# facebookresearch/multimodal

Measured on NVIDIA H100. Metric: image-text pairs/sec (CLIP ViT-B/16 contrastive pretrain step, bs=512/GPU), higher is better.
Workload: dtype bf16

## Files before the change

### multimodal_b200/csrc/attention.cu

```cuda
#include "attention_tiles.cuh"
#include "mmb200_internal.h"
#include <stdlib.h>

namespace mmb {

constexpr int SMAX = 384;

__device__ __forceinline__ void load_tile(uint8_t* dst, const __nv_bfloat16* src, long long ld, int S, int S_pad) {
  for (int i = threadIdx.x; i < S_pad * 8; i += blockDim.x) {
    const int r = i >> 3, ch = i & 7;
    uint4 v = make_uint4(0, 0, 0, 0);
    if (r < S) v = __ldg(reinterpret_cast<const uint4*>(src + (long long)r * ld + ch * 8));
    *reinterpret_cast<uint4*>(dst + toff(r, ch * 8)) = v;
  }
}
__device__ __forceinline__ void cp_tile_rows(uint8_t* dst, const __nv_bfloat16* src, long long ld, int S, int r0,
                                             int r1) {
  for (int i = r0 * 8 + threadIdx.x; i < r1 * 8; i += blockDim.x) {
    const int r = i >> 3, ch = i & 7;
    const bool in = r < S;
    cp_async16(smem_u32(dst + toff(r, ch * 8)), src + (in ? (long long)r * ld + ch * 8 : 0), in ? 16u : 0u);
  }
}

__device__ __forceinline__ void load_keymask(uint8_t* dst, const uint8_t* kmask, int S, int S_pad) {
  for (int i = threadIdx.x; i < S_pad; i += blockDim.x) dst[i] = (i < S && (!kmask || kmask[i])) ? 1 : 0;
}

template <bool CAUSAL>
__global__ void __launch_bounds__(256) attn_fwd_kernel(const __nv_bfloat16* __restrict__ qkv,
                                                       __nv_bfloat16* __restrict__ out, float* __restrict__ lse,
                                                       const uint8_t* __restrict__ kmask, int S, int H,
                                                       float scale_log2) {
  extern __shared__ __align__(128) uint8_t asmem[];
  const int S_pad = (S + 15) & ~15;
  const int d = H * HD;
  const long long ld = 3LL * d;
  const int b = blockIdx.x / H, h = blockIdx.x - b * H;
  uint8_t* sQ = asmem;
  uint8_t* sK = sQ + S_pad * 128;
  uint8_t* sV = sK + S_pad * 128;
  uint64_t* bars = reinterpret_cast<uint64_t*>(sV + S_pad * 128);
  uint8_t* sM = reinterpret_cast<uint8_t*>(bars + SMAX / 64);
  const __nv_bfloat16* base = qkv + (long long)b * S * ld + h * HD;
  const int n_kc = (S_pad + 63) >> 6;
  if (threadIdx.x == 0)
    for (int c = 0; c < n_kc; ++c) mbar_init(&bars[c], blockDim.x);
  load_keymask(sM, kmask ? kmask + (long long)b * S : nullptr, S, S_pad);
  __syncthreads();
  cp_tile_rows(sQ, base, ld, S, 0, S_pad);
  for (int c = 0; c < n_kc; ++c) {
    const int k1 = min(S_pad, (c + 1) * 64);
    cp_tile_rows(sK, base + d, ld, S, c * 64, k1);
    cp_tile_rows(sV, base + 2 * d, ld, S, c * 64, k1);
    cp_async_arrive(&bars[c]);
  }
  const uint32_t uQ = smem_u32(sQ), uK = smem_u32(sK), uV = smem_u32(sV);
  const int warp = threadIdx.x >> 5, lane = threadIdx.x & 31, nwarps = blockDim.x >> 5;
  const int g = lane >> 2, t = lane & 3;
  const int n_qt = S_pad >> 4;
  mbar_wait_quiet(&bars[0], 0);

  for (int qt = warp; qt < n_qt; qt += nwarps) {
    const int q0 = qt * 16;
    uint32_t qa[4][4];
#pragma unroll
    for (int ks = 0; ks < 4; ++ks) load_a(qa[ks], uQ, q0, ks * 16, lane);
    float o[8][4];
#pragma unroll
    for (int i = 0; i < 8; ++i) o[i][0] = o[i][1] = o[i][2] = o[i][3] = 0.f;
    float m0 = -INFINITY, m1 = -INFINITY, l0 = 0.f, l1 = 0.f;
    const int r0 = q0 + g, r1 = r0 + 8;
    const int kv_end = CAUSAL ? min(S, q0 + 16) : S;

    for (int kvb = 0; kvb < kv_end; kvb += 64) {
      mbar_wait_quiet(&bars[kvb >> 6], 0);
      const int nt_valid = min(8, (kv_end - kvb + 7) >> 3);
      float s[8][4];
#pragma unroll
      for (int nt = 0; nt < 8; ++nt) {
        s[nt][0] = s[nt][1] = s[nt][2] = s[nt][3] = 0.f;
        if (nt < nt_valid) {
#pragma unroll
          for (int kp = 0; kp < 2; ++kp) {
            uint32_t kb[4];
            load_b_nk(kb, uK, kvb + nt * 8, kp * 32, lane);
            mma16816(s[nt], qa[2 * kp], kb[0], kb[1]);
            mma16816(s[nt], qa[2 * kp + 1], kb[2], kb[3]);
          }
        }
      }
      float mx0 = -INFINITY, mx1 = -INFINITY;
#pragma unroll
      for (int nt = 0; nt < 8; ++nt) {
#pragma unroll
        for (int e = 0; e < 4; ++e) {
          const int col = kvb + nt * 8 + 2 * t + (e & 1);
          const int row = (e < 2) ? r0 : r1;
          float v = s[nt][e] * scale_log2;
          if (col >= kv_end || !sM[col] || (CAUSAL && col > row)) v = -INFINITY;
          s[nt][e] = v;
        }
        mx0 = fmaxf(mx0, fmaxf(s[nt][0], s[nt][1]));
        mx1 = fmaxf(mx1, fmaxf(s[nt][2], s[nt][3]));
      }
      mx0 = quad_max(mx0);
      mx1 = quad_max(mx1);
      const float mn0 = fmaxf(m0, mx0), mn1 = fmaxf(m1, mx1);
      const float b0 = (mn0 == -INFINITY) ? 0.f : mn0, b1 = (mn1 == -INFINITY) ? 0.f : mn1;
      const float c0 = exp2f(m0 - b0), c1 = exp2f(m1 - b1);
      float rs0 = 0.f, rs1 = 0.f;
#pragma unroll
      for (int nt = 0; nt < 8; ++nt) {
        s[nt][0] = exp2f(s[nt][0] - b0);
        s[nt][1] = exp2f(s[nt][1] - b0);
        s[nt][2] = exp2f(s[nt][2] - b1);
        s[nt][3] = exp2f(s[nt][3] - b1);
        rs0 += s[nt][0] + s[nt][1];
        rs1 += s[nt][2] + s[nt][3];
      }
      l0 = l0 * c0 + rs0;
      l1 = l1 * c1 + rs1;
      m0 = mn0;
      m1 = mn1;
#pragma unroll
      for (int i = 0; i < 8; ++i) {
        o[i][0] *= c0; o[i][1] *= c0; o[i][2] *= c1; o[i][3] *= c1;
      }
#pragma unroll
      for (int ks = 0; ks < 4; ++ks) {
        if (2 * ks < nt_valid) {
          uint32_t pa[4];
          pa[0] = pack_bf16x2(s[2 * ks][0], s[2 * ks][1]);
          pa[1] = pack_bf16x2(s[2 * ks][2], s[2 * ks][3]);
          pa[2] = pack_bf16x2(s[2 * ks + 1][0], s[2 * ks + 1][1]);
          pa[3] = pack_bf16x2(s[2 * ks + 1][2], s[2 * ks + 1][3]);
#pragma unroll
          for (int np = 0; np < 4; ++np) {
            uint32_t vb[4];
            load_b_kn(vb, uV, kvb + ks * 16, np * 16, lane);
            mma16816(o[2 * np], pa, vb[0], vb[1]);
            mma16816(o[2 * np + 1], pa, vb[2], vb[3]);
          }
        }
      }
    }
    l0 = quad_sum(l0);
    l1 = quad_sum(l1);
    const float i0 = l0 > 0.f ? 1.f / l0 : 0.f, i1 = l1 > 0.f ? 1.f / l1 : 0.f;
    __nv_bfloat16* orow0 = out + ((long long)b * S + r0) * d + h * HD;
    __nv_bfloat16* orow1 = out + ((long long)b * S + r1) * d + h * HD;
#pragma unroll
    for (int nt = 0; nt < 8; ++nt) {
      if (r0 < S) *reinterpret_cast<uint32_t*>(orow0 + nt * 8 + 2 * t) = pack_bf16x2(o[nt][0] * i0, o[nt][1] * i0);
      if (r1 < S) *reinterpret_cast<uint32_t*>(orow1 + nt * 8 + 2 * t) = pack_bf16x2(o[nt][2] * i1, o[nt][3] * i1);
    }
    if (lse && t == 0) {
      float* lrow = lse + ((long long)b * H + h) * S;
      if (r0 < S) lrow[r0] = (m0 + log2f(l0)) * 0.6931471805599453f;
      if (r1 < S) lrow[r1] = (m1 + log2f(l1)) * 0.6931471805599453f;
    }
  }
  cp_async_wait_all();
}

template <bool CAUSAL>
__global__ void __launch_bounds__(256) attn_bwd_kernel(const __nv_bfloat16* __restrict__ qkv,
                                                       const __nv_bfloat16* __restrict__ out,
                                                       const __nv_bfloat16* __restrict__ dout,
                                                       const float* __restrict__ lse,
                                                       const uint8_t* __restrict__ kmask,
                                                       __nv_bfloat16* __restrict__ dqkv, int S, int H, float scale) {
  extern __shared__ __align__(128) uint8_t asmem[];
  const int S_pad = (S + 15) & ~15;
  const int d = H * HD;
  const long long ld = 3LL * d;
  const int b = blockIdx.x / H, h = blockIdx.x - b * H;
  uint8_t* sQ = asmem;
  uint8_t* sK = sQ + S_pad * 128;
  uint8_t* sV = sK + S_pad * 128;
  uint8_t* sdO = sV + S_pad * 128;
  float* sL = reinterpret_cast<float*>(sdO + S_pad * 128);
  float* sD = sL + S_pad;
  uint8_t* sM = reinterpret_cast<uint8_t*>(sD + S_pad);
  const __nv_bfloat16* base = qkv + (long long)b * S * ld + h * HD;
  const __nv_bfloat16* obase = out + (long long)b * S * d + h * HD;
  const __nv_bfloat16* dobase = dout + (long long)b * S * d + h * HD;
  load_tile(sQ, base, ld, S, S_pad);
  load_tile(sK, base + d, ld, S, S_pad);
  load_tile(sV, base + 2 * d, ld, S, S_pad);
  load_tile(sdO, dobase, d, S, S_pad);
  load_keymask(sM, kmask ? kmask + (long long)b * S : nullptr, S, S_pad);
  const int warp = threadIdx.x >> 5, lane = threadIdx.x & 31, nwarps = blockDim.x >> 5;
  for (int r = warp; r < S_pad; r += nwarps) {
    float acc = 0.f;
    if (r < S) {
      const uint32_t a = *reinterpret_cast<const uint32_t*>(obase + (long long)r * d + lane * 2);
      const uint32_t c = *reinterpret_cast<const uint32_t*>(dobase + (long long)r * d + lane * 2);
      acc = bf16_lo(a) * bf16_lo(c) + bf16_hi(a) * bf16_hi(c);
    }
#pragma unroll
    for (int o = 16; o > 0; o >>= 1) acc += __shfl_xor_sync(0xffffffffu, acc, o);
    if (lane == 0) {
      sD[r] = acc;
      sL[r] = (r < S) ? lse[((long long)b * H + h) * S + r] * 1.4426950408889634f : 0.f;
    }
  }
  __syncthreads();
  const uint32_t uQ = smem_u32(sQ), uK = smem_u32(sK), uV = smem_u32(sV), uO = smem_u32(sdO);
  const int g = lane >> 2, t = lane & 3;
  const int n_t = S_pad >> 4;
  const float scale_log2 = scale * 1.4426950408889634f;
  __nv_bfloat16* dbase = dqkv + (long long)b * S * ld + h * HD;

  for (int j = warp; j < n_t; j += nwarps) {
    const int kv0 = j * 16;
    uint32_t ka[4][4], va[4][4];
#pragma unroll
    for (int ks = 0; ks < 4; ++ks) {
      load_a(ka[ks], uK, kv0, ks * 16, lane);
      load_a(va[ks], uV, kv0, ks * 16, lane);
    }
    float dk[8][4], dv[8][4];
#pragma unroll
    for (int i = 0; i < 8; ++i) {
      dk[i][0] = dk[i][1] = dk[i][2] = dk[i][3] = 0.f;
      dv[i][0] = dv[i][1] = dv[i][2] = dv[i][3] = 0.f;
    }
    const bool kv_ok0 = sM[kv0 + g] != 0, kv_ok1 = sM[kv0 + g + 8] != 0;
    for (int i = CAUSAL ? j : 0; i < n_t; ++i) {
      const int q0 = i * 16;
      float st[2][4], dpt[2][4];
#pragma unroll
      for (int nt = 0; nt < 2; ++nt) {
        st[nt][0] = st[nt][1] = st[nt][2] = st[nt][3] = 0.f;
        dpt[nt][0] = dpt[nt][1] = dpt[nt][2] = dpt[nt][3] = 0.f;
#pragma unroll
        for (int kp = 0; kp < 2; ++kp) {
          uint32_t qb[4], ob[4];
          load_b_nk(qb, uQ, q0 + nt * 8, kp * 32, lane);
          mma16816(st[nt], ka[2 * kp], qb[0], qb[1]);
          mma16816(st[nt], ka[2 * kp + 1], qb[2], qb[3]);
          load_b_nk(ob, uO, q0 + nt * 8, kp * 32, lane);
          mma16816(dpt[nt], va[2 * kp], ob[0], ob[1]);
          mma16816(dpt[nt], va[2 * kp + 1], ob[2], ob[3]);
        }
      }
      float pT[2][4], dsT[2][4];
#pragma unroll
      for (int nt = 0; nt < 2; ++nt)
#pragma unroll
        for (int e = 0; e < 4; ++e) {
          const int kv = kv0 + g + (e >> 1) * 8;
          const int q = q0 + nt * 8 + 2 * t + (e & 1);
          const bool valid = ((e >> 1) ? kv_ok1 : kv_ok0) && (q < S) && (!CAUSAL || kv <= q);
          const float p = valid ? exp2f(st[nt][e] * scale_log2 - sL[q]) : 0.f;
          pT[nt][e] = p;
          dsT[nt][e] = p * (dpt[nt][e] - sD[q]) * scale;
        }
      uint32_t pa[4], dsa[4];
      pa[0] = pack_bf16x2(pT[0][0], pT[0][1]); pa[1] = pack_bf16x2(pT[0][2], pT[0][3]);
      pa[2] = pack_bf16x2(pT[1][0], pT[1][1]); pa[3] = pack_bf16x2(pT[1][2], pT[1][3]);
      dsa[0] = pack_bf16x2(dsT[0][0], dsT[0][1]); dsa[1] = pack_bf16x2(dsT[0][2], dsT[0][3]);
      dsa[2] = pack_bf16x2(dsT[1][0], dsT[1][1]); dsa[3] = pack_bf16x2(dsT[1][2], dsT[1][3]);
#pragma unroll
      for (int np = 0; np < 4; ++np) {
        uint32_t bb[4];
        load_b_kn(bb, uO, q0, np * 16, lane);
        mma16816(dv[2 * np], pa, bb[0], bb[1]);
        mma16816(dv[2 * np + 1], pa, bb[2], bb[3]);
        load_b_kn(bb, uQ, q0, np * 16, lane);
        mma16816(dk[2 * np], dsa, bb[0], bb[1]);
        mma16816(dk[2 * np + 1], dsa, bb[2], bb[3]);
      }
    }
    const int r0 = kv0 + g, r1 = r0 + 8;
#pragma unroll
    for (int nt = 0; nt < 8; ++nt) {
      if (r0 < S) {
        *reinterpret_cast<uint32_t*>(dbase + (long long)r0 * ld + d + nt * 8 + 2 * t) = pack_bf16x2(dk[nt][0], dk[nt][1]);
        *reinterpret_cast<uint32_t*>(dbase + (long long)r0 * ld + 2 * d + nt * 8 + 2 * t) = pack_bf16x2(dv[nt][0], dv[nt][1]);
      }
      if (r1 < S) {
        *reinterpret_cast<uint32_t*>(dbase + (long long)r1 * ld + d + nt * 8 + 2 * t) = pack_bf16x2(dk[nt][2], dk[nt][3]);
        *reinterpret_cast<uint32_t*>(dbase + (long long)r1 * ld + 2 * d + nt * 8 + 2 * t) = pack_bf16x2(dv[nt][2], dv[nt][3]);
      }
    }
  }

  for (int i = warp; i < n_t; i += nwarps) {
    const int q0 = i * 16;
    uint32_t qa[4][4], oa[4][4];
#pragma unroll
    for (int ks = 0; ks < 4; ++ks) {
      load_a(qa[ks], uQ, q0, ks * 16, lane);
      load_a(oa[ks], uO, q0, ks * 16, lane);
    }
    float dq[8][4];
#pragma unroll
    for (int n = 0; n < 8; ++n) dq[n][0] = dq[n][1] = dq[n][2] = dq[n][3] = 0.f;
    const int r0 = q0 + g, r1 = r0 + 8;
    const float L0 = sL[r0], L1 = sL[r1], D0 = sD[r0], D1 = sD[r1];
    const int j_end = CAUSAL ? i + 1 : n_t;
    for (int j = 0; j < j_end; ++j) {
      const int kv0 = j * 16;
      float s[2][4], dp[2][4];
#pragma unroll
      for (int nt = 0; nt < 2; ++nt) {
        s[nt][0] = s[nt][1] = s[nt][2] = s[nt][3] = 0.f;
        dp[nt][0] = dp[nt][1] = dp[nt][2] = dp[nt][3] = 0.f;
#pragma unroll
        for (int kp = 0; kp < 2; ++kp) {
          uint32_t kb[4], vb[4];
          load_b_nk(kb, uK, kv0 + nt * 8, kp * 32, lane);
          mma16816(s[nt], qa[2 * kp], kb[0], kb[1]);
          mma16816(s[nt], qa[2 * kp + 1], kb[2], kb[3]);
          load_b_nk(vb, uV, kv0 + nt * 8, kp * 32, lane);
          mma16816(dp[nt], oa[2 * kp], vb[0], vb[1]);
          mma16816(dp[nt], oa[2 * kp + 1], vb[2], vb[3]);
        }
      }
      float ds[2][4];
#pragma unroll
      for (int nt = 0; nt < 2; ++nt)
#pragma unroll
        for (int e = 0; e < 4; ++e) {
          const int row = (e < 2) ? r0 : r1;
          const int col = kv0 + nt * 8 + 2 * t + (e & 1);
          const bool valid = (row < S) && sM[col] && (!CAUSAL || col <= row);
          const float p = valid ? exp2f(s[nt][e] * scale_log2 - ((e < 2) ? L0 : L1)) : 0.f;
          ds[nt][e] = p * (dp[nt][e] - ((e < 2) ? D0 : D1)) * scale;
        }
      uint32_t dsa[4];
      dsa[0] = pack_bf16x2(ds[0][0], ds[0][1]); dsa[1] = pack_bf16x2(ds[0][2], ds[0][3]);
      dsa[2] = pack_bf16x2(ds[1][0], ds[1][1]); dsa[3] = pack_bf16x2(ds[1][2], ds[1][3]);
#pragma unroll
      for (int np = 0; np < 4; ++np) {
        uint32_t bb[4];
        load_b_kn(bb, uK, kv0, np * 16, lane);
        mma16816(dq[2 * np], dsa, bb[0], bb[1]);
        mma16816(dq[2 * np + 1], dsa, bb[2], bb[3]);
      }
    }
#pragma unroll
    for (int nt = 0; nt < 8; ++nt) {
      if (r0 < S) *reinterpret_cast<uint32_t*>(dbase + (long long)r0 * ld + nt * 8 + 2 * t) = pack_bf16x2(dq[nt][0], dq[nt][1]);
      if (r1 < S) *reinterpret_cast<uint32_t*>(dbase + (long long)r1 * ld + nt * 8 + 2 * t) = pack_bf16x2(dq[nt][2], dq[nt][3]);
    }
  }
}

constexpr int BWD_STAGED_MAX = 224;
constexpr int BWD_STAGED_THREADS = BWD_STAGED_MAX / 16 * 32;
constexpr int BWD_STAGED_BARS = 1 + (BWD_STAGED_MAX + 63) / 64;

__host__ __device__ constexpr int ds_stride(int S_pad) { return 2 * S_pad + 16; }
__host__ __device__ constexpr int bwd_staged_smem(int S_pad) {
  return 4 * S_pad * 128 + S_pad * ds_stride(S_pad) + 2 * S_pad * 4 + 8 * BWD_STAGED_BARS + S_pad;
}
static_assert(bwd_staged_smem(BWD_STAGED_MAX) <= 227 * 1024, "staged backward exceeds the sm_90 shared-memory opt-in");

template <bool CAUSAL>
__global__ void __launch_bounds__(BWD_STAGED_THREADS, 1) attn_bwd_staged_kernel(
    const __nv_bfloat16* __restrict__ qkv, const __nv_bfloat16* __restrict__ out, const __nv_bfloat16* __restrict__ dout,
    const float* __restrict__ lse, const uint8_t* __restrict__ kmask, __nv_bfloat16* __restrict__ dqkv, int S, int H,
    float scale) {
  extern __shared__ __align__(128) uint8_t asmem[];
  const int S_pad = (S + 15) & ~15;
  const int dstride = ds_stride(S_pad);
  const int d = H * HD;
  const long long ld = 3LL * d;
  const int b = blockIdx.x / H, h = blockIdx.x - b * H;
  uint8_t* sQ = asmem;
  uint8_t* sK = sQ + S_pad * 128;
  uint8_t* sV = sK + S_pad * 128;
  uint8_t* sdO = sV + S_pad * 128;
  uint8_t* sdS = sdO + S_pad * 128;
  float* sL = reinterpret_cast<float*>(sdS + S_pad * dstride);
  float* sD = sL + S_pad;
  uint64_t* bars = reinterpret_cast<uint64_t*>(sD + S_pad);
  uint8_t* sM = reinterpret_cast<uint8_t*>(bars + BWD_STAGED_BARS);
  const __nv_bfloat16* base = qkv + (long long)b * S * ld + h * HD;
  const __nv_bfloat16* obase = out + (long long)b * S * d + h * HD;
  const __nv_bfloat16* dobase = dout + (long long)b * S * d + h * HD;
  const int n_qc = (S_pad + 63) >> 6;
  if (threadIdx.x == 0)
    for (int c = 0; c <= n_qc; ++c) mbar_init(&bars[c], blockDim.x);
  load_keymask(sM, kmask ? kmask + (long long)b * S : nullptr, S, S_pad);
  __syncthreads();
  cp_tile_rows(sK, base + d, ld, S, 0, S_pad);
  cp_tile_rows(sV, base + 2 * d, ld, S, 0, S_pad);
  cp_async_arrive(&bars[0]);
  for (int c = 0; c < n_qc; ++c) {
    const int q1 = min(S_pad, (c + 1) * 64);
    cp_tile_rows(sQ, base, ld, S, c * 64, q1);
    cp_tile_rows(sdO, dobase, d, S, c * 64, q1);
    cp_async_arrive(&bars[1 + c]);
  }
  for (int r = threadIdx.x >> 3; r < S_pad; r += blockDim.x >> 3) {
    const int ch = threadIdx.x & 7;
    float v[4] = {0.f, 0.f, 0.f, 0.f};
    if (r < S) {
      const uint4 a = __ldg(reinterpret_cast<const uint4*>(obase + (long long)r * d + ch * 8));
      const uint4 c = __ldg(reinterpret_cast<const uint4*>(dobase + (long long)r * d + ch * 8));
      v[0] = bf16_lo(a.x) * bf16_lo(c.x) + bf16_hi(a.x) * bf16_hi(c.x);
      v[1] = bf16_lo(a.y) * bf16_lo(c.y) + bf16_hi(a.y) * bf16_hi(c.y);
      v[2] = bf16_lo(a.z) * bf16_lo(c.z) + bf16_hi(a.z) * bf16_hi(c.z);
      v[3] = bf16_lo(a.w) * bf16_lo(c.w) + bf16_hi(a.w) * bf16_hi(c.w);
    }
#pragma unroll
    for (int o = 4; o > 0; o >>= 1)
#pragma unroll
      for (int k = 0; k < 4; ++k) v[k] += __shfl_xor_sync(0xffffffffu, v[k], o);
    if (ch == 0) {
      sD[r] = (v[0] + v[2]) + (v[1] + v[3]);
      sL[r] = (r < S) ? lse[((long long)b * H + h) * S + r] * 1.4426950408889634f : 0.f;
    }
  }
  __syncthreads();
  const uint32_t uQ = smem_u32(sQ), uK = smem_u32(sK), uV = smem_u32(sV), uO = smem_u32(sdO), udS = smem_u32(sdS);
  const int warp = threadIdx.x >> 5, lane = threadIdx.x & 31;
  const int g = lane >> 2, t = lane & 3;
  const int n_t = S_pad >> 4;
  const float scale_log2 = scale * 1.4426950408889634f;
  __nv_bfloat16* dbase = dqkv + (long long)b * S * ld + h * HD;

  {
    const int j = warp, kv0 = j * 16;
    mbar_wait_quiet(&bars[0], 0);
    float dk[8][4], dv[8][4];
#pragma unroll
    for (int i = 0; i < 8; ++i) {
      dk[i][0] = dk[i][1] = dk[i][2] = dk[i][3] = 0.f;
      dv[i][0] = dv[i][1] = dv[i][2] = dv[i][3] = 0.f;
    }
    const bool kv_ok0 = sM[kv0 + g] != 0, kv_ok1 = sM[kv0 + g + 8] != 0;
    const int i0 = CAUSAL ? j : 0;
#pragma unroll 1
    for (int i = i0; i < n_t; ++i) {
      while (!mbar_try_wait(&bars[1 + (i >> 2)], 0)) {}
      const int q0 = i * 16;
      float st[2][4], dpt[2][4];
#pragma unroll
      for (int nt = 0; nt < 2; ++nt) {
        st[nt][0] = st[nt][1] = st[nt][2] = st[nt][3] = 0.f;
        dpt[nt][0] = dpt[nt][1] = dpt[nt][2] = dpt[nt][3] = 0.f;
      }
#pragma unroll
      for (int kp = 0; kp < 2; ++kp) {
        uint32_t ka0[4], ka1[4];
        load_a(ka0, uK, kv0, kp * 32, lane);
        load_a(ka1, uK, kv0, kp * 32 + 16, lane);
#pragma unroll
        for (int nt = 0; nt < 2; ++nt) {
          uint32_t qb[4];
          load_b_nk(qb, uQ, q0 + nt * 8, kp * 32, lane);
          mma16816(st[nt], ka0, qb[0], qb[1]);
          mma16816(st[nt], ka1, qb[2], qb[3]);
        }
      }
#pragma unroll
      for (int kp = 0; kp < 2; ++kp) {
        uint32_t va0[4], va1[4];
        load_a(va0, uV, kv0, kp * 32, lane);
        load_a(va1, uV, kv0, kp * 32 + 16, lane);
#pragma unroll
        for (int nt = 0; nt < 2; ++nt) {
          uint32_t ob[4];
          load_b_nk(ob, uO, q0 + nt * 8, kp * 32, lane);
          mma16816(dpt[nt], va0, ob[0], ob[1]);
          mma16816(dpt[nt], va1, ob[2], ob[3]);
        }
      }
      float pT[2][4], dsT[2][4];
#pragma unroll
      for (int nt = 0; nt < 2; ++nt)
#pragma unroll
        for (int e = 0; e < 4; ++e) {
          const int kv = kv0 + g + (e >> 1) * 8;
          const int q = q0 + nt * 8 + 2 * t + (e & 1);
          const bool valid = ((e >> 1) ? kv_ok1 : kv_ok0) && (q < S) && (!CAUSAL || kv <= q);
          const float p = valid ? exp2f(st[nt][e] * scale_log2 - sL[q]) : 0.f;
          pT[nt][e] = p;
          dsT[nt][e] = p * (dpt[nt][e] - sD[q]) * scale;
        }
      uint32_t pa[4], dsa[4];
      pa[0] = pack_bf16x2(pT[0][0], pT[0][1]); pa[1] = pack_bf16x2(pT[0][2], pT[0][3]);
      pa[2] = pack_bf16x2(pT[1][0], pT[1][1]); pa[3] = pack_bf16x2(pT[1][2], pT[1][3]);
      dsa[0] = pack_bf16x2(dsT[0][0], dsT[0][1]); dsa[1] = pack_bf16x2(dsT[0][2], dsT[0][3]);
      dsa[2] = pack_bf16x2(dsT[1][0], dsT[1][1]); dsa[3] = pack_bf16x2(dsT[1][2], dsT[1][3]);
      uint8_t* ds_row0 = sdS + (kv0 + g) * dstride + (q0 + 2 * t) * 2;
      *reinterpret_cast<uint32_t*>(ds_row0) = dsa[0];
      *reinterpret_cast<uint32_t*>(ds_row0 + 8 * dstride) = dsa[1];
      *reinterpret_cast<uint32_t*>(ds_row0 + 16) = dsa[2];
      *reinterpret_cast<uint32_t*>(ds_row0 + 8 * dstride + 16) = dsa[3];
#pragma unroll
      for (int np = 0; np < 4; ++np) {
        uint32_t bb[4];
        load_b_kn(bb, uO, q0, np * 16, lane);
        mma16816(dv[2 * np], pa, bb[0], bb[1]);
        mma16816(dv[2 * np + 1], pa, bb[2], bb[3]);
        load_b_kn(bb, uQ, q0, np * 16, lane);
        mma16816(dk[2 * np], dsa, bb[0], bb[1]);
        mma16816(dk[2 * np + 1], dsa, bb[2], bb[3]);
      }
    }
    const int r0 = kv0 + g, r1 = r0 + 8;
#pragma unroll
    for (int nt = 0; nt < 8; ++nt) {
      if (r0 < S) {
        *reinterpret_cast<uint32_t*>(dbase + (long long)r0 * ld + d + nt * 8 + 2 * t) = pack_bf16x2(dk[nt][0], dk[nt][1]);
        *reinterpret_cast<uint32_t*>(dbase + (long long)r0 * ld + 2 * d + nt * 8 + 2 * t) = pack_bf16x2(dv[nt][0], dv[nt][1]);
      }
      if (r1 < S) {
        *reinterpret_cast<uint32_t*>(dbase + (long long)r1 * ld + d + nt * 8 + 2 * t) = pack_bf16x2(dk[nt][2], dk[nt][3]);
        *reinterpret_cast<uint32_t*>(dbase + (long long)r1 * ld + 2 * d + nt * 8 + 2 * t) = pack_bf16x2(dv[nt][2], dv[nt][3]);
      }
    }
  }
  cp_async_wait_all();
  __syncthreads();

  {
    const int i = warp, q0 = i * 16;
    float dq[8][4];
#pragma unroll
    for (int n = 0; n < 8; ++n) dq[n][0] = dq[n][1] = dq[n][2] = dq[n][3] = 0.f;
    const uint32_t ds_lane = udS + ((lane & 7) + ((lane >> 4) & 1) * 8) * dstride + (q0 + ((lane >> 3) & 1) * 8) * 2;
    const int j_end = CAUSAL ? i + 1 : n_t;
    for (int j = 0; j < j_end; ++j) {
      const int kv0 = j * 16;
      uint32_t dsa[4];
      ldsm_x4_t(dsa, ds_lane + kv0 * dstride);
#pragma unroll
      for (int np = 0; np < 4; ++np) {
        uint32_t bb[4];
        load_b_kn(bb, uK, kv0, np * 16, lane);
        mma16816(dq[2 * np], dsa, bb[0], bb[1]);
        mma16816(dq[2 * np + 1], dsa, bb[2], bb[3]);
      }
    }
    const int r0 = q0 + g, r1 = r0 + 8;
#pragma unroll
    for (int nt = 0; nt < 8; ++nt) {
      if (r0 < S) *reinterpret_cast<uint32_t*>(dbase + (long long)r0 * ld + nt * 8 + 2 * t) = pack_bf16x2(dq[nt][0], dq[nt][1]);
      if (r1 < S) *reinterpret_cast<uint32_t*>(dbase + (long long)r1 * ld + nt * 8 + 2 * t) = pack_bf16x2(dq[nt][2], dq[nt][3]);
    }
  }
}

static int pick_threads(int S) {
  const int n_t = (S + 15) / 16;
  const int per = (n_t + 7) / 8;
  return ((n_t + per - 1) / per) * 32;
}

static int attention_fwd_impl(const void* qkv, void* out, float* lse, const uint8_t* kmask, int B, int S, int H,
                              int causal, float scale, void* stream) {
  if (B <= 0 || S <= 0 || H <= 0) return MMB_ERR_UNSUPPORTED;
  if (S > SMAX)
    return attention_fwd_stream(qkv, out, lse, kmask, B, S, H, causal, scale, reinterpret_cast<cudaStream_t>(stream));
  const int S_pad = (S + 15) & ~15;
  const int smem = 3 * S_pad * 128 + 8 * (SMAX / 64) + S_pad;
  const float scale_log2 = scale * 1.4426950408889634f;
  cudaStream_t st = reinterpret_cast<cudaStream_t>(stream);
  auto kfn = causal ? attn_fwd_kernel<true> : attn_fwd_kernel<false>;
  cudaError_t e = cudaFuncSetAttribute(kfn, cudaFuncAttributeMaxDynamicSharedMemorySize, smem);
  if (e != cudaSuccess) return (int)e;
  kfn<<<B * H, pick_threads(S), smem, st>>>((const __nv_bfloat16*)qkv, (__nv_bfloat16*)out, lse, kmask, S, H, scale_log2);
  return (int)cudaGetLastError();
}

static int attention_bwd_impl(const void* qkv, const void* out, const void* dout, const float* lse, void* dqkv,
                              const uint8_t* kmask, int B, int S, int H, int causal, float scale, void* stream) {
  if (B <= 0 || S <= 0 || H <= 0) return MMB_ERR_UNSUPPORTED;
  if (S > SMAX)
    return attention_bwd_stream(qkv, out, dout, lse, dqkv, kmask, B, S, H, causal, scale,
                                reinterpret_cast<cudaStream_t>(stream));
  const int S_pad = (S + 15) & ~15;
  cudaStream_t st = reinterpret_cast<cudaStream_t>(stream);
  if (S_pad <= BWD_STAGED_MAX) {
    const int smem = bwd_staged_smem(S_pad);
    auto kfn = causal ? attn_bwd_staged_kernel<true> : attn_bwd_staged_kernel<false>;
    cudaError_t e = cudaFuncSetAttribute(kfn, cudaFuncAttributeMaxDynamicSharedMemorySize, smem);
    if (e != cudaSuccess) return (int)e;
    kfn<<<B * H, (S_pad / 16) * 32, smem, st>>>((const __nv_bfloat16*)qkv, (const __nv_bfloat16*)out,
                                                (const __nv_bfloat16*)dout, lse, kmask, (__nv_bfloat16*)dqkv, S, H, scale);
    return (int)cudaGetLastError();
  }
  const int smem = 4 * S_pad * 128 + 2 * S_pad * 4 + S_pad;
  auto kfn = causal ? attn_bwd_kernel<true> : attn_bwd_kernel<false>;
  cudaError_t e = cudaFuncSetAttribute(kfn, cudaFuncAttributeMaxDynamicSharedMemorySize, smem);
  if (e != cudaSuccess) return (int)e;
  kfn<<<B * H, pick_threads(S), smem, st>>>((const __nv_bfloat16*)qkv, (const __nv_bfloat16*)out,
                                            (const __nv_bfloat16*)dout, lse, kmask, (__nv_bfloat16*)dqkv, S, H, scale);
  return (int)cudaGetLastError();
}

}

using namespace mmb;

extern "C" int mmb_attention_bwd_launches(int S) { return S > SMAX ? ATTN_BWD_STREAM_LAUNCHES : 1; }

extern "C" int mmb_attention_fwd(const void* qkv, void* out, float* lse, int B, int S, int H, int head_dim, int causal,
                                 float scale, void* stream) {
  if (head_dim != HD) return MMB_ERR_UNSUPPORTED;
  return attention_fwd_impl(qkv, out, lse, nullptr, B, S, H, causal, scale, stream);
}
extern "C" int mmb_attention_fwd_kmask(const void* qkv, void* out, float* lse, const unsigned char* kmask, int B, int S,
                                       int H, int head_dim, int causal, float scale, void* stream) {
  if (head_dim != HD) return MMB_ERR_UNSUPPORTED;
  return attention_fwd_impl(qkv, out, lse, kmask, B, S, H, causal, scale, stream);
}
extern "C" int mmb_attention_bwd(const void* qkv, const void* out, const void* dout, const float* lse, void* dqkv,
                                 int B, int S, int H, int head_dim, int causal, float scale, void* stream) {
  if (head_dim != HD) return MMB_ERR_UNSUPPORTED;
  return attention_bwd_impl(qkv, out, dout, lse, dqkv, nullptr, B, S, H, causal, scale, stream);
}
extern "C" int mmb_attention_bwd_kmask(const void* qkv, const void* out, const void* dout, const float* lse, void* dqkv,
                                       const unsigned char* kmask, int B, int S, int H, int head_dim, int causal,
                                       float scale, void* stream) {
  if (head_dim != HD) return MMB_ERR_UNSUPPORTED;
  return attention_bwd_impl(qkv, out, dout, lse, dqkv, kmask, B, S, H, causal, scale, stream);
}
```

Measured before the change: 3078.

## Make staged attention backward persistent with cross-head prefetch of K/V/dO

Converts the staged attention backward kernel into a persistent kernel sized to SM occupancy, with each block looping over heads. K, V and dO for the next head are loaded asynchronously while the current head's dQ is computed, Q and K share a ping-pong buffer, and L2 prefetch is issued for the next head's output and LSE rows. The aim is to hide per-block global load latency and launch tail, at the cost of more complex phase-tracked barrier logic and serialized per-head work within a block.

```diff
diff --git a/multimodal_b200/csrc/attention.cu b/multimodal_b200/csrc/attention.cu
--- a/multimodal_b200/csrc/attention.cu
+++ b/multimodal_b200/csrc/attention.cu
@@ -360,43 +360,8 @@
 }
 static_assert(bwd_staged_smem(BWD_STAGED_MAX) <= 227 * 1024, "staged backward exceeds the sm_90 shared-memory opt-in");
 
-template <bool CAUSAL>
-__global__ void __launch_bounds__(BWD_STAGED_THREADS, 1) attn_bwd_staged_kernel(
-    const __nv_bfloat16* __restrict__ qkv, const __nv_bfloat16* __restrict__ out, const __nv_bfloat16* __restrict__ dout,
-    const float* __restrict__ lse, const uint8_t* __restrict__ kmask, __nv_bfloat16* __restrict__ dqkv, int S, int H,
-    float scale) {
-  extern __shared__ __align__(128) uint8_t asmem[];
-  const int S_pad = (S + 15) & ~15;
-  const int dstride = ds_stride(S_pad);
-  const int d = H * HD;
-  const long long ld = 3LL * d;
-  const int b = blockIdx.x / H, h = blockIdx.x - b * H;
-  uint8_t* sQ = asmem;
-  uint8_t* sK = sQ + S_pad * 128;
-  uint8_t* sV = sK + S_pad * 128;
-  uint8_t* sdO = sV + S_pad * 128;
-  uint8_t* sdS = sdO + S_pad * 128;
-  float* sL = reinterpret_cast<float*>(sdS + S_pad * dstride);
-  float* sD = sL + S_pad;
-  uint64_t* bars = reinterpret_cast<uint64_t*>(sD + S_pad);
-  uint8_t* sM = reinterpret_cast<uint8_t*>(bars + BWD_STAGED_BARS);
-  const __nv_bfloat16* base = qkv + (long long)b * S * ld + h * HD;
-  const __nv_bfloat16* obase = out + (long long)b * S * d + h * HD;
-  const __nv_bfloat16* dobase = dout + (long long)b * S * d + h * HD;
-  const int n_qc = (S_pad + 63) >> 6;
-  if (threadIdx.x == 0)
-    for (int c = 0; c <= n_qc; ++c) mbar_init(&bars[c], blockDim.x);
-  load_keymask(sM, kmask ? kmask + (long long)b * S : nullptr, S, S_pad);
-  __syncthreads();
-  cp_tile_rows(sK, base + d, ld, S, 0, S_pad);
-  cp_tile_rows(sV, base + 2 * d, ld, S, 0, S_pad);
-  cp_async_arrive(&bars[0]);
-  for (int c = 0; c < n_qc; ++c) {
-    const int q1 = min(S_pad, (c + 1) * 64);
-    cp_tile_rows(sQ, base, ld, S, c * 64, q1);
-    cp_tile_rows(sdO, dobase, d, S, c * 64, q1);
-    cp_async_arrive(&bars[1 + c]);
-  }
+__device__ __forceinline__ void bwd_rows_d_l(float* sD, float* sL, const __nv_bfloat16* obase,
+                                            const __nv_bfloat16* dobase, const float* lrow, int d, int S, int S_pad) {
   for (int r = threadIdx.x >> 3; r < S_pad; r += blockDim.x >> 3) {
     const int ch = threadIdx.x & 7;
     float v[4] = {0.f, 0.f, 0.f, 0.f};
@@ -414,139 +379,221 @@
       for (int k = 0; k < 4; ++k) v[k] += __shfl_xor_sync(0xffffffffu, v[k], o);
     if (ch == 0) {
       sD[r] = (v[0] + v[2]) + (v[1] + v[3]);
-      sL[r] = (r < S) ? lse[((long long)b * H + h) * S + r] * 1.4426950408889634f : 0.f;
-    }
-  }
-  __syncthreads();
-  const uint32_t uQ = smem_u32(sQ), uK = smem_u32(sK), uV = smem_u32(sV), uO = smem_u32(sdO), udS = smem_u32(sdS);
+      sL[r] = (r < S) ? lrow[r] * 1.4426950408889634f : 0.f;
+    }
+  }
+}
+__device__ __forceinline__ void prefetch_l2(const void* p) { asm volatile("prefetch.global.L2 [%0];" ::"l"(p)); }
+
+template <bool CAUSAL>
+__global__ void __launch_bounds__(BWD_STAGED_THREADS, 1) attn_bwd_staged_kernel(
+    const __nv_bfloat16* __restrict__ qkv, const __nv_bfloat16* __restrict__ out, const __nv_bfloat16* __restrict__ dout,
+    const float* __restrict__ lse, const uint8_t* __restrict__ kmask, __nv_bfloat16* __restrict__ dqkv, int S, int H,
+    int BH, float scale) {
+  extern __shared__ __align__(128) uint8_t asmem[];
+  const int S_pad = (S + 15) & ~15;
+  const int dstride = ds_stride(S_pad);
+  const int d = H * HD;
+  const long long ld = 3LL * d;
+  uint8_t* sQK = asmem;
+  uint8_t* sV = sQK + 2 * S_pad * 128;
+  uint8_t* sdO = sV + S_pad * 128;
+  uint8_t* sdS = sdO + S_pad * 128;
+  float* sL = reinterpret_cast<float*>(sdS + S_pad * dstride);
+  float* sD = sL + S_pad;
+  uint64_t* bars = reinterpret_cast<uint64_t*>(sD + S_pad);
+  uint8_t* sM = reinterpret_cast<uint8_t*>(bars + BWD_STAGED_BARS);
+  const int n_qc = (S_pad + 63) >> 6;
   const int warp = threadIdx.x >> 5, lane = threadIdx.x & 31;
   const int g = lane >> 2, t = lane & 3;
   const int n_t = S_pad >> 4;
   const float scale_log2 = scale * 1.4426950408889634f;
-  __nv_bfloat16* dbase = dqkv + (long long)b * S * ld + h * HD;
-
-  {
-    const int j = warp, kv0 = j * 16;
-    mbar_wait_quiet(&bars[0], 0);
-    float dk[8][4], dv[8][4];
-#pragma unroll
-    for (int i = 0; i < 8; ++i) {
-      dk[i][0] = dk[i][1] = dk[i][2] = dk[i][3] = 0.f;
-      dv[i][0] = dv[i][1] = dv[i][2] = dv[i][3] = 0.f;
-    }
-    const bool kv_ok0 = sM[kv0 + g] != 0, kv_ok1 = sM[kv0 + g + 8] != 0;
-    const int i0 = CAUSAL ? j : 0;
+  auto qkv_of = [&](int hd) { return qkv + (long long)(hd / H) * S * ld + (hd % H) * HD; };
+  auto od_of = [&](const __nv_bfloat16* p, int hd) { return p + (long long)(hd / H) * S * d + (hd % H) * HD; };
+  auto mask_of = [&](int hd) { return kmask ? kmask + (long long)(hd / H) * S : nullptr; };
+  auto load_kvo = [&](uint8_t* dK, int hd) {
+    cp_tile_rows(dK, qkv_of(hd) + d, ld, S, 0, S_pad);
+    cp_tile_rows(sV, qkv_of(hd) + 2 * d, ld, S, 0, S_pad);
+    cp_tile_rows(sdO, od_of(dout, hd), d, S, 0, S_pad);
+    cp_async_arrive(&bars[0]);
+  };
+  auto load_q = [&](uint8_t* dQ, int hd) {
+    for (int c = 0; c < n_qc; ++c) {
+      cp_tile_rows(dQ, qkv_of(hd), ld, S, c * 64, min(S_pad, (c + 1) * 64));
+      cp_async_arrive(&bars[1 + c]);
+    }
+  };
+
+  if (threadIdx.x == 0)
+    for (int c = 0; c <= n_qc; ++c) mbar_init(&bars[c], blockDim.x);
+  load_keymask(sM, mask_of(blockIdx.x), S, S_pad);
+  __syncthreads();
+  load_kvo(sQK + S_pad * 128, blockIdx.x);
+  load_q(sQK, blockIdx.x);
+  bwd_rows_d_l(sD, sL, od_of(out, blockIdx.x), od_of(dout, blockIdx.x), lse + (long long)blockIdx.x * S, d, S, S_pad);
+  __syncthreads();
+
+  uint32_t phase = 0;
+  for (int hd = blockIdx.x; hd < BH; hd += gridDim.x) {
+    const int next = hd + gridDim.x;
+    const bool more = next < BH;
+    uint8_t* const sQ = sQK + phase * (S_pad * 128);
+    uint8_t* const sK = sQK + (phase ^ 1) * (S_pad * 128);
+    const uint32_t uQ = smem_u32(sQ), uK = smem_u32(sK), uV = smem_u32(sV), uO = smem_u32(sdO), udS = smem_u32(sdS);
+
+    {
+      const int j = warp, kv0 = j * 16;
+      mbar_wait_quiet(&bars[0], phase);
+      float dk[8][4], dv[8][4];
+#pragma unroll
+      for (int i = 0; i < 8; ++i) {
+        dk[i][0] = dk[i][1] = dk[i][2] = dk[i][3] = 0.f;
+        dv[i][0] = dv[i][1] = dv[i][2] = dv[i][3] = 0.f;
+      }
+      const bool kv_ok0 = sM[kv0 + g] != 0, kv_ok1 = sM[kv0 + g + 8] != 0;
+      const int i0 = CAUSAL ? j : 0;
 #pragma unroll 1
-    for (int i = i0; i < n_t; ++i) {
-      while (!mbar_try_wait(&bars[1 + (i >> 2)], 0)) {}
-      const int q0 = i * 16;
-      float st[2][4], dpt[2][4];
-#pragma unroll
-      for (int nt = 0; nt < 2; ++nt) {
-        st[nt][0] = st[nt][1] = st[nt][2] = st[nt][3] = 0.f;
-        dpt[nt][0] = dpt[nt][1] = dpt[nt][2] = dpt[nt][3] = 0.f;
-      }
-#pragma unroll
-      for (int kp = 0; kp < 2; ++kp) {
-        uint32_t ka0[4], ka1[4];
-        load_a(ka0, uK, kv0, kp * 32, lane);
-        load_a(ka1, uK, kv0, kp * 32 + 16, lane);
+      for (int i = i0; i < n_t; ++i) {
+        mbar_wait_quiet(&bars[1 + (i >> 2)], phase);
+        const int q0 = i * 16;
+        float st[2][4], dpt[2][4];
 #pragma unroll
         for (int nt = 0; nt < 2; ++nt) {
-          uint32_t qb[4];
-          load_b_nk(qb, uQ, q0 + nt * 8, kp * 32, lane);
-          mma16816(st[nt], ka0, qb[0], qb[1]);
-          mma16816(st[nt], ka1, qb[2], qb[3]);
-        }
-      }
-#pragma unroll
-      for (int kp = 0; kp < 2; ++kp) {
-        uint32_t va0[4], va1[4];
-        load_a(va0, uV, kv0, kp * 32, lane);
-        load_a(va1, uV, kv0, kp * 32 + 16, lane);
-#pragma unroll
-        for (int nt = 0; nt < 2; ++nt) {
-          uint32_t ob[4];
-          load_b_nk(ob, uO, q0 + nt * 8, kp * 32, lane);
-          mma16816(dpt[nt], va0, ob[0], ob[1]);
-          mma16816(dpt[nt], va1, ob[2], ob[3]);
-        }
-      }
-      float pT[2][4], dsT[2][4];
-#pragma unroll
-      for (int nt = 0; nt < 2; ++nt)
-#pragma unroll
-        for (int e = 0; e < 4; ++e) {
-          const int kv = kv0 + g + (e >> 1) * 8;
-          const int q = q0 + nt * 8 + 2 * t + (e & 1);
-          const bool valid = ((e >> 1) ? kv_ok1 : kv_ok0) && (q < S) && (!CAUSAL || kv <= q);
-          const float p = valid ? exp2f(st[nt][e] * scale_log2 - sL[q]) : 0.f;
-          pT[nt][e] = p;
-          dsT[nt][e] = p * (dpt[nt][e] - sD[q]) * scale;
-        }
-      uint32_t pa[4], dsa[4];
-      pa[0] = pack_bf16x2(pT[0][0], pT[0][1]); pa[1] = pack_bf16x2(pT[0][2], pT[0][3]);
-      pa[2] = pack_bf16x2(pT[1][0], pT[1][1]); pa[3] = pack_bf16x2(pT[1][2], pT[1][3]);
-      dsa[0] = pack_bf16x2(dsT[0][0], dsT[0][1]); dsa[1] = pack_bf16x2(dsT[0][2], dsT[0][3]);
-      dsa[2] = pack_bf16x2(dsT[1][0], dsT[1][1]); dsa[3] = pack_bf16x2(dsT[1][2], dsT[1][3]);
-      uint8_t* ds_row0 = sdS + (kv0 + g) * dstride + (q0 + 2 * t) * 2;
-      *reinterpret_cast<uint32_t*>(ds_row0) = dsa[0];
-      *reinterpret_cast<uint32_t*>(ds_row0 + 8 * dstride) = dsa[1];
-      *reinterpret_cast<uint32_t*>(ds_row0 + 16) = dsa[2];
-      *reinterpret_cast<uint32_t*>(ds_row0 + 8 * dstride + 16) = dsa[3];
-#pragma unroll
-      for (int np = 0; np < 4; ++np) {
-        uint32_t bb[4];
-        load_b_kn(bb, uO, q0, np * 16, lane);
-        mma16816(dv[2 * np], pa, bb[0], bb[1]);
-        mma16816(dv[2 * np + 1], pa, bb[2], bb[3]);
-        load_b_kn(bb, uQ, q0, np * 16, lane);
-        mma16816(dk[2 * np], dsa, bb[0], bb[1]);
-        mma16816(dk[2 * np + 1], dsa, bb[2], bb[3]);
-      }
-    }
-    const int r0 = kv0 + g, r1 = r0 + 8;
-#pragma unroll
-    for (int nt = 0; nt < 8; ++nt) {
-      if (r0 < S) {
-        *reinterpret_cast<uint32_t*>(dbase + (long long)r0 * ld + d + nt * 8 + 2 * t) = pack_bf16x2(dk[nt][0], dk[nt][1]);
-        *reinterpret_cast<uint32_t*>(dbase + (long long)r0 * ld + 2 * d + nt * 8 + 2 * t) = pack_bf16x2(dv[nt][0], dv[nt][1]);
-      }
-      if (r1 < S) {
-        *reinterpret_cast<uint32_t*>(dbase + (long long)r1 * ld + d + nt * 8 + 2 * t) = pack_bf16x2(dk[nt][2], dk[nt][3]);
-        *reinterpret_cast<uint32_t*>(dbase + (long long)r1 * ld + 2 * d + nt * 8 + 2 * t) = pack_bf16x2(dv[nt][2], dv[nt][3]);
-      }
-    }
-  }
-  cp_async_wait_all();
-  __syncthreads();
-
-  {
-    const int i = warp, q0 = i * 16;
-    float dq[8][4];
-#pragma unroll
-    for (int n = 0; n < 8; ++n) dq[n][0] = dq[n][1] = dq[n][2] = dq[n][3] = 0.f;
-    const uint32_t ds_lane = udS + ((lane & 7) + ((lane >> 4) & 1) * 8) * dstride + (q0 + ((lane >> 3) & 1) * 8) * 2;
-    const int j_end = CAUSAL ? i + 1 : n_t;
-    for (int j = 0; j < j_end; ++j) {
-      const int kv0 = j * 16;
-      uint32_t dsa[4];
-      ldsm_x4_t(dsa, ds_lane + kv0 * dstride);
-#pragma unroll
-      for (int np = 0; np < 4; ++np) {
-        uint32_t bb[4];
-        load_b_kn(bb, uK, kv0, np * 16, lane);
-        mma16816(dq[2 * np], dsa, bb[0], bb[1]);
-        mma16816(dq[2 * np + 1], dsa, bb[2], bb[3]);
-      }
-    }
-    const int r0 = q0 + g, r1 = r0 + 8;
-#pragma unroll
-    for (int nt = 0; nt < 8; ++nt) {
-      if (r0 < S) *reinterpret_cast<uint32_t*>(dbase + (long long)r0 * ld + nt * 8 + 2 * t) = pack_bf16x2(dq[nt][0], dq[nt][1]);
-      if (r1 < S) *reinterpret_cast<uint32_t*>(dbase + (long long)r1 * ld + nt * 8 + 2 * t) = pack_bf16x2(dq[nt][2], dq[nt][3]);
-    }
-  }
+          st[nt][0] = st[nt][1] = st[nt][2] = st[nt][3] = 0.f;
+          dpt[nt][0] = dpt[nt][1] = dpt[nt][2] = dpt[nt][3] = 0.f;
+        }
+#pragma unroll
+        for (int kp = 0; kp < 2; ++kp) {
+          uint32_t ka0[4], ka1[4];
+          load_a(ka0, uK, kv0, kp * 32, lane);
+          load_a(ka1, uK, kv0, kp * 32 + 16, lane);
+#pragma unroll
+          for (int nt = 0; nt < 2; ++nt) {
+            uint32_t qb[4];
+            load_b_nk(qb, uQ, q0 + nt * 8, kp * 32, lane);
+            mma16816(st[nt], ka0, qb[0], qb[1]);
+            mma16816(st[nt], ka1, qb[2], qb[3]);
+          }
+        }
+#pragma unroll
+        for (int kp = 0; kp < 2; ++kp) {
+          uint32_t va0[4], va1[4];
+          load_a(va0, uV, kv0, kp * 32, lane);
+          load_a(va1, uV, kv0, kp * 32 + 16, lane);
+#pragma unroll
+          for (int nt = 0; nt < 2; ++nt) {
+            uint32_t ob[4];
+            load_b_nk(ob, uO, q0 + nt * 8, kp * 32, lane);
+            mma16816(dpt[nt], va0, ob[0], ob[1]);
+            mma16816(dpt[nt], va1, ob[2], ob[3]);
+          }
+        }
+        float pT[2][4], dsT[2][4];
+#pragma unroll
+        for (int nt = 0; nt < 2; ++nt)
+#pragma unroll
+          for (int e = 0; e < 4; ++e) {
+            const int kv = kv0 + g + (e >> 1) * 8;
+            const int q = q0 + nt * 8 + 2 * t + (e & 1);
+            const bool valid = ((e >> 1) ? kv_ok1 : kv_ok0) && (q < S) && (!CAUSAL || kv <= q);
+            const float p = valid ? exp2f(st[nt][e] * scale_log2 - sL[q]) : 0.f;
+            pT[nt][e] = p;
+            dsT[nt][e] = p * (dpt[nt][e] - sD[q]) * scale;
+          }
+        uint32_t pa[4], dsa[4];
+        pa[0] = pack_bf16x2(pT[0][0], pT[0][1]); pa[1] = pack_bf16x2(pT[0][2], pT[0][3]);
+        pa[2] = pack_bf16x2(pT[1][0], pT[1][1]); pa[3] = pack_bf16x2(pT[1][2], pT[1][3]);
+        dsa[0] = pack_bf16x2(dsT[0][0], dsT[0][1]); dsa[1] = pack_bf16x2(dsT[0][2], dsT[0][3]);
+        dsa[2] = pack_bf16x2(dsT[1][0], dsT[1][1]); dsa[3] = pack_bf16x2(dsT[1][2], dsT[1][3]);
+        uint8_t* ds_row0 = sdS + (kv0 + g) * dstride + (q0 + 2 * t) * 2;
+        *reinterpret_cast<uint32_t*>(ds_row0) = dsa[0];
+        *reinterpret_cast<uint32_t*>(ds_row0 + 8 * dstride) = dsa[1];
+        *reinterpret_cast<uint32_t*>(ds_row0 + 16) = dsa[2];
+        *reinterpret_cast<uint32_t*>(ds_row0 + 8 * dstride + 16) = dsa[3];
+#pragma unroll
+        for (int np = 0; np < 4; ++np) {
+          uint32_t bb[4];
+          load_b_kn(bb, uO, q0, np * 16, lane);
+          mma16816(dv[2 * np], pa, bb[0], bb[1]);
+          mma16816(dv[2 * np + 1], pa, bb[2], bb[3]);
+          load_b_kn(bb, uQ, q0, np * 16, lane);
+          mma16816(dk[2 * np], dsa, bb[0], bb[1]);
+          mma16816(dk[2 * np + 1], dsa, bb[2], bb[3]);
+        }
+      }
+      const int r0 = kv0 + g, r1 = r0 + 8;
+      __nv_bfloat16* const dbase = dqkv + (long long)(hd / H) * S * ld + (hd % H) * HD;
+#pragma unroll
+      for (int nt = 0; nt < 8; ++nt) {
+        if (r0 < S) {
+          *reinterpret_cast<uint32_t*>(dbase + (long long)r0 * ld + d + nt * 8 + 2 * t) = pack_bf16x2(dk[nt][0], dk[nt][1]);
+          *reinterpret_cast<uint32_t*>(dbase + (long long)r0 * ld + 2 * d + nt * 8 + 2 * t) = pack_bf16x2(dv[nt][0], dv[nt][1]);
+        }
+        if (r1 < S) {
+          *reinterpret_cast<uint32_t*>(dbase + (long long)r1 * ld + d + nt * 8 + 2 * t) = pack_bf16x2(dk[nt][2], dk[nt][3]);
+          *reinterpret_cast<uint32_t*>(dbase + (long long)r1 * ld + 2 * d + nt * 8 + 2 * t) = pack_bf16x2(dv[nt][2], dv[nt][3]);
+        }
+      }
+    }
+    __syncthreads();
+
+    uint8_t next_mask = 0;
+    if (more) {
+      load_kvo(sQ, next);
+      for (int r = threadIdx.x; r < S; r += blockDim.x) prefetch_l2(od_of(out, next) + (long long)r * d);
+      if (threadIdx.x < (S + 31) / 32) prefetch_l2(lse + (long long)next * S + threadIdx.x * 32);
+      const uint8_t* m = mask_of(next);
+      if (threadIdx.x < S) next_mask = (!m || m[threadIdx.x]) ? 1 : 0;
+    }
+
+    {
+      const int i = warp, q0 = i * 16;
+      float dq[8][4];
+#pragma unroll
+      for (int n = 0; n < 8; ++n) dq[n][0] = dq[n][1] = dq[n][2] = dq[n][3] = 0.f;
+      const uint32_t ds_lane = udS + ((lane & 7) + ((lane >> 4) & 1) * 8) * dstride + (q0 + ((lane >> 3) & 1) * 8) * 2;
+      const int j_end = CAUSAL ? i + 1 : n_t;
+      for (int j = 0; j < j_end; ++j) {
+        const int kv0 = j * 16;
+        uint32_t dsa[4];
+        ldsm_x4_t(dsa, ds_lane + kv0 * dstride);
+#pragma unroll
+        for (int np = 0; np < 4; ++np) {
+          uint32_t bb[4];
+          load_b_kn(bb, uK, kv0, np * 16, lane);
+          mma16816(dq[2 * np], dsa, bb[0], bb[1]);
+          mma16816(dq[2 * np + 1], dsa, bb[2], bb[3]);
+        }
+      }
+      const int r0 = q0 + g, r1 = r0 + 8;
+      __nv_bfloat16* const dbase = dqkv + (long long)(hd / H) * S * ld + (hd % H) * HD;
+#pragma unroll
+      for (int nt = 0; nt < 8; ++nt) {
+        if (r0 < S) *reinterpret_cast<uint32_t*>(dbase + (long long)r0 * ld + nt * 8 + 2 * t) = pack_bf16x2(dq[nt][0], dq[nt][1]);
+        if (r1 < S) *reinterpret_cast<uint32_t*>(dbase + (long long)r1 * ld + nt * 8 + 2 * t) = pack_bf16x2(dq[nt][2], dq[nt][3]);
+      }
+    }
+
+    if (more) {
+      bwd_rows_d_l(sD, sL, od_of(out, next), od_of(dout, next), lse + (long long)next * S, d, S, S_pad);
+      if (threadIdx.x < S_pad) sM[threadIdx.x] = next_mask;
+    }
+    __syncthreads();
+    if (more) load_q(sK, next);
+    phase ^= 1;
+  }
+}
+
+template <typename K>
+static cudaError_t persistent_grid(K kfn, int threads, int smem, int heads, int* grid) {
+  int dev = 0, sms = 0, per_sm = 0;
+  cudaError_t e = cudaGetDevice(&dev);
+  if (e == cudaSuccess) e = cudaDeviceGetAttribute(&sms, cudaDevAttrMultiProcessorCount, dev);
+  if (e == cudaSuccess) e = cudaOccupancyMaxActiveBlocksPerMultiprocessor(&per_sm, kfn, threads, smem);
+  if (e != cudaSuccess) return e;
+  if (per_sm < 1) return cudaErrorInvalidConfiguration;
+  *grid = heads < sms * per_sm ? heads : sms * per_sm;
+  return cudaSuccess;
 }
 
 static int pick_threads(int S) {
@@ -580,12 +627,15 @@
   const int S_pad = (S + 15) & ~15;
   cudaStream_t st = reinterpret_cast<cudaStream_t>(stream);
   if (S_pad <= BWD_STAGED_MAX) {
-    const int smem = bwd_staged_smem(S_pad);
+    const int smem = bwd_staged_smem(S_pad), threads = (S_pad / 16) * 32;
     auto kfn = causal ? attn_bwd_staged_kernel<true> : attn_bwd_staged_kernel<false>;
     cudaError_t e = cudaFuncSetAttribute(kfn, cudaFuncAttributeMaxDynamicSharedMemorySize, smem);
     if (e != cudaSuccess) return (int)e;
-    kfn<<<B * H, (S_pad / 16) * 32, smem, st>>>((const __nv_bfloat16*)qkv, (const __nv_bfloat16*)out,
-                                                (const __nv_bfloat16*)dout, lse, kmask, (__nv_bfloat16*)dqkv, S, H, scale);
+    int grid = 0;
+    e = persistent_grid(kfn, threads, smem, B * H, &grid);
+    if (e != cudaSuccess) return (int)e;
+    kfn<<<grid, threads, smem, st>>>((const __nv_bfloat16*)qkv, (const __nv_bfloat16*)out, (const __nv_bfloat16*)dout,
+                                     lse, kmask, (__nv_bfloat16*)dqkv, S, H, B * H, scale);
     return (int)cudaGetLastError();
   }
   const int smem = 4 * S_pad * 128 + 2 * S_pad * 4 + S_pad;
```

After: 3109 (median of 6 runs). 1.01x the previous value.
